# sm00thix/cvmatrix

Hardware: AMD Instinct MI355X
Metric: folds/sec (training_XTX_XTY, center+scale) at N=1e5,K=512 (higher is better)
Workload: dtype f64

## Files before the change

### cvmatrix_amd/csrc/wgram4.hpp

```cpp
#pragma once

constexpr int NT4 = 512;
template <typename T> __device__ __forceinline__ void partial_store(T *p, T v) { *p = v; }
constexpr int NBUF4 = 4;
constexpr size_t LDS4_BYTES = (size_t)NBUF4 * BUF_ELEMS * 8;
template <typename T> constexpr size_t lds4_bytes() { return (size_t)NBUF4 * BUF_ELEMS * sizeof(T); }

__host__ __device__ inline size_t fstat_len(int K, int M);
template <typename T> struct FusedPre;
template <typename T>
__device__ __forceinline__ void fused_g_preload32(FusedPre<T> &p, int a0, int b0, int K, const T *Gt, int lane, int row_lo);
template <typename T, int TP>
__device__ __forceinline__ void fused_finish_direct32(T (*Ts)[TP], const double *rs, int a0, int b0, int K, T *out,
                                                      double swt, bool cX, bool sX, int lane, int row_lo,
                                                      const FusedPre<T> &p);
template <typename T, int TP>
__device__ __forceinline__ void fused_finish_block(T (*Ts)[TP], const double *rs, bool diagb, int a0,
                                                   int b0, int K, const T *Gt, T *out,
                                                   double swt, bool cX, bool sX, int lane);
template <typename T, int TP>
__device__ __forceinline__ void fused_finish_direct(T (*Ts)[TP], const double *rs, bool diagb, int a0,
                                                    int b0, int K, const T *Gt, T *out,
                                                    double swt, bool cX, bool sX, int lane, int row_lo, int row_hi);
template <typename T, int TP>
// ... 96 lines not shown
  else { seg_begin = 0; seg_rows = a.N; }
  int64_t r0, r1;
  split_range(seg_rows, wi.nsp, sp, r0, r1);
  r0 = uni64(r0); r1 = uni64(r1); seg_begin = uni64(seg_begin);
  const int nstages = uni((int)((r1 - r0 + STAGE_ROWS - 1) / STAGE_ROWS));
  const int colA0 = uni(ti * TILE), colB0 = uni(tj * TILE);

  if (ROLER == 3) {
    const int d = wave_all - 4;
    const char *zero_src = reinterpret_cast<const char *>(unip(g_zero_line));
    constexpr unsigned ES = sizeof(T);
    constexpr int EPL = 16 / (int)ES;
    const char *one_src = reinterpret_cast<const char *>(ES == 8 ? (const void *)unip(g_one_line)
                                                                : (const void *)unip(g_one_line_f));
    int oa = EPL * lane, ob = EPL * lane, oy = ES == 8 ? 2 * (lane & 15) : (lane & 31);
    if (colA0 + oa > g.K - EPL) oa = g.K - EPL - colA0;
    if (colB0 + ob > g.K - EPL) ob = g.K - EPL - colB0;
    if (oa < 0) oa = 0;
    if (ob < 0) ob = 0;
    const int ycol0 = yc * YT;
    const int ylast = ES == 8 ? g.M - 2 : g.M - 1;
    if (g.M > 0) { if (ycol0 + oy > ylast) oy = ylast - ycol0; if (oy < 0) oy = 0; } else oy = 0;
    const unsigned va = ES * (unsigned)oa, vb = ES * (unsigned)ob, vy = ES * (unsigned)oy, vw = 4u * (unsigned)lane;
    const unsigned lds0 = (unsigned)(uintptr_t)((__attribute__((address_space(3))) char *)smem_raw);
    auto dma16_all = [&](const char *sbase, unsigned voff, unsigned lds_addr) {
      unsigned keep;
      asm volatile("s_mov_b32 %0, m0\n\ts_mov_b32 m0, %3\n\ts_nop 0\n\t"
                   "global_load_lds_dwordx4 %1, %2\n\ts_mov_b32 m0, %0"
                   : "=&s"(keep) : "v"(voff), "s"(sbase), "s"(lds_addr) : "memory");
    };
    auto dma16_lo16 = [&](const char *sbase, unsigned voff, unsigned lds_addr) {
      unsigned keep; unsigned long long ex;
      asm volatile("s_mov_b32 %0, m0\n\ts_mov_b64 %1, exec\n\ts_mov_b64 exec, 0xffff\n\ts_mov_b32 m0, %4\n\ts_nop 0\n\t"
                   "global_load_lds_dwordx4 %2, %3\n\ts_mov_b64 exec, %1\n\ts_mov_b32 m0, %0"
                   : "=&s"(keep), "=&s"(ex) : "v"(voff), "s"(sbase), "s"(lds_addr) : "memory");
    };
    auto dma16_lo32 = [&](const char *sbase, unsigned voff, unsigned lds_addr) {
      unsigned keep; unsigned long long ex;
      asm volatile("s_mov_b32 %0, m0\n\ts_mov_b64 %1, exec\n\ts_mov_b64 exec, 0xffffffff\n\ts_mov_b32 m0, %4\n\ts_nop 0\n\t"
                   "global_load_lds_dwordx4 %2, %3\n\ts_mov_b64 exec, %1\n\ts_mov_b32 m0, %0"
                   : "=&s"(keep), "=&s"(ex) : "v"(voff), "s"(sbase), "s"(lds_addr) : "memory");
    };
    auto dma4_lo32 = [&](const char *sbase, unsigned voff, unsigned lds_addr) {
      unsigned keep; unsigned long long ex;
      asm volatile("s_mov_b32 %0, m0\n\ts_mov_b64 %1, exec\n\ts_mov_b64 exec, 0xffffffff\n\ts_mov_b32 m0, %4\n\ts_nop 0\n\t"
                   "global_load_lds_dword %2, %3\n\ts_mov_b64 exec, %1\n\ts_mov_b32 m0, %0"
                   : "=&s"(keep), "=&s"(ex) : "v"(voff), "s"(sbase), "s"(lds_addr) : "memory");
    };
    auto dma4_lo1 = [&](const char *sbase, unsigned voff, unsigned lds_addr) {
      unsigned keep; unsigned long long ex;
      asm volatile("s_mov_b32 %0, m0\n\ts_mov_b64 %1, exec\n\ts_mov_b64 exec, 1\n\ts_mov_b32 m0, %4\n\ts_nop 0\n\t"
                   "global_load_lds_dword %2, %3\n\ts_mov_b64 exec, %1\n\ts_mov_b32 m0, %0"
                   : "=&s"(keep), "=&s"(ex) : "v"(voff), "s"(sbase), "s"(lds_addr) : "memory");
    };
    auto dma4_lo2 = [&](const char *sbase, unsigned voff, unsigned lds_addr) {
      unsigned keep; unsigned long long ex;
      asm volatile("s_mov_b32 %0, m0\n\ts_mov_b64 %1, exec\n\ts_mov_b64 exec, 3\n\ts_mov_b32 m0, %4\n\ts_nop 0\n\t"
                   "global_load_lds_dword %2, %3\n\ts_mov_b64 exec, %1\n\ts_mov_b32 m0, %0"
                   : "=&s"(keep), "=&s"(ex) : "v"(voff), "s"(sbase), "s"(lds_addr) : "memory");
    };
    const int r0i = uni((int)r0), r1i = uni((int)r1);
    auto row_numbers = [&](int t, int64_t (&rn)[4], bool (&ok)[4]) {
      int rr[4];
#pragma unroll
      for (int j = 0; j < 4; ++j) {
        rr[j] = r0i + t * STAGE_ROWS + d + 4 * j;
        ok[j] = rr[j] < r1i;
      }
      if (!GATHER) {
#pragma unroll
        for (int j = 0; j < 4; ++j) rn[j] = seg_begin + rr[j];
        return;
      }
      const int64_t *p0 = a.idx + seg_begin + (ok[0] ? rr[0] : 0);
      const int64_t *p1 = a.idx + seg_begin + (ok[1] ? rr[1] : 0);
      const int64_t *p2 = a.idx + seg_begin + (ok[2] ? rr[2] : 0);
      const int64_t *p3 = a.idx + seg_begin + (ok[3] ? rr[3] : 0);
      int64_t v0 = 0, v1 = 0, v2 = 0, v3 = 0;
      if (r1i > 0) {
        asm volatile("s_load_dwordx2 %0, %4, 0x0\n\ts_load_dwordx2 %1, %5, 0x0\n\t"
                     "s_load_dwordx2 %2, %6, 0x0\n\ts_load_dwordx2 %3, %7, 0x0\n\t"
                     "s_waitcnt lgkmcnt(0)"
                     : "=&s"(v0), "=&s"(v1), "=&s"(v2), "=&s"(v3)
                     : "s"(p0), "s"(p1), "s"(p2), "s"(p3) : "memory");
      }
      rn[0] = v0; rn[1] = v1; rn[2] = v2; rn[3] = v3;
    };
    auto issue_stage = [&](int t, const int64_t (&rn)[4], const bool (&ok)[4]) {
      const unsigned bufb = lds0 + (unsigned)((t % NBUF4) * BUF_ELEMS) * ES;
#pragma unroll
      for (int j = 0; j < 4; ++j) {
        const int lrow = d + 4 * j;
        const bool valid = ok[j];
        const char *xrow = reinterpret_cast<const char *>(a.X + rn[j] * (int64_t)g.K);
        const char *pa = valid ? xrow + (int64_t)ES * colA0 : zero_src;
        if (ES == 8) dma16_all(pa, va, bufb + (unsigned)(lrow * PITCH) * ES);
        else dma16_lo32(pa, va, bufb + (unsigned)(lrow * PITCH) * ES);
        if (!diag) {
          const char *pb = valid ? xrow + (int64_t)ES * colB0 : zero_src;
          if (ES == 8) dma16_all(pb, vb, bufb + (unsigned)(PANEL_ELEMS + lrow * PITCH) * ES);
          else dma16_lo32(pb, vb, bufb + (unsigned)(PANEL_ELEMS + lrow * PITCH) * ES);
        } else {
          const char *yrow = (valid && g.M > 0)
              ? reinterpret_cast<const char *>(a.Y + rn[j] * (int64_t)g.M + ycol0) : zero_src;
          if (ES == 8) dma16_lo16(yrow, vy, bufb + (unsigned)(PANEL_ELEMS + lrow * YPITCH) * ES);
          else dma4_lo32(yrow, vy, bufb + (unsigned)(PANEL_ELEMS + lrow * YPITCH) * ES);
        }
        const char *wsrc = valid ? (WEIGHTED ? reinterpret_cast<const char *>(a.w + rn[j]) : one_src) : zero_src;
        if (ES == 8) dma4_lo2(wsrc, vw, bufb + (unsigned)(2 * PANEL_ELEMS + lrow) * ES);
        else dma4_lo1(wsrc, vw, bufb + (unsigned)(2 * PANEL_ELEMS + lrow) * ES);
      }
    };
    auto wait_one_stage_in_flight = [&]() { asm volatile("s_waitcnt vmcnt(12)" ::: "memory"); };
    int64_t rn[4];
    bool ok[4];
#pragma unroll
    for (int t = 0; t < 3; ++t) {
      row_numbers(t, rn, ok);
      issue_stage(t, rn, ok);
    }
    wait_one_stage_in_flight();
    __builtin_amdgcn_s_barrier();
    __builtin_amdgcn_s_barrier();
#ifdef CVM_STAMPS
    unsigned long long t_a = 0, t_b = 0, t_c = 0, t0, t1, t2, t3;
#endif
#pragma unroll 1
    for (int s = 0; s < nstages; ++s) {
#ifdef CVM_STAMPS
      STAMP(t0);
#endif
      row_numbers(s + 3, rn, ok);
      issue_stage(s + 3, rn, ok);
#ifdef CVM_STAMPS
      STAMP(t1);
#endif
      wait_one_stage_in_flight();
#ifdef CVM_STAMPS
      STAMP(t2);
#endif
#ifdef CVM_STAMPS
      if (!(a.dbg & 4))
#endif
      __builtin_amdgcn_s_barrier();
#ifdef CVM_STAMPS
      STAMP(t3);
      t_a += t1 - t0; t_b += t2 - t1; t_c += t3 - t2;
#endif
    }
    asm volatile("s_waitcnt vmcnt(0) lgkmcnt(0)" ::: "memory");
    if constexpr (FUSEDR) {
      if (a.stat_flags && do_g && !diag && d == 0) {
        const int *fl = a.stat_flags + (size_t)seg * g.P;
        fused_wait_flag<T>(fl + ti, fl + tj, smem_raw, lane, seg, uni(xcd_q), uni(slot_q), a.fused_status,
                           a.retry_items, a.retry_mode, a.test_mode);
      }
    }
    if (FUSEDR) lds_barrier();
    if constexpr (FUSEDR) {
      if (do_g && diag && a.stat_flags) {
        __builtin_amdgcn_s_barrier();
        __builtin_amdgcn_s_barrier();
        if (d == 0) {
          const int K = g.K, M = g.M;
          double *fsw = const_cast<double *>(a.fstats) + (size_t)seg * fstat_len(K, M);
          const double *stl = reinterpret_cast<const double *>(smem_raw + diag_tile_bytes<T>()) + 768;
#pragma unroll
          for (int h = 0; h < 2; ++h) {
            const int lcol = 64 * h + lane, col = ti * TILE + lcol;
            if (col < K) { stc(fsw + col, stl[lcol]); stc(fsw + K + col, stl[128 + lcol]); }
          }
          if (lane < 32 && lane < M) { stc(fsw + 2 * K + lane, stl[256 + lane]); stc(fsw + 2 * K + M + lane, stl[288 + lane]); }
          if (lane == 0) stc(fsw + 2 * K + 2 * M, stl[320]);
          asm volatile("s_waitcnt vmcnt(0)" ::: "memory");
          if (lane == 0)
            __hip_atomic_store(a.stat_flags + (size_t)seg * g.P + ti, 1, __ATOMIC_RELAXED, __HIP_MEMORY_SCOPE_AGENT);
        }
      }
      if (do_g && diag && a.out_XTX) {
        constexpr int TP = TILE + 1;
        const int K = g.K, M = g.M;
        const double *fs = a.fstats + (size_t)seg * fstat_len(K, M);
        const double swt = a.stat_flags ? (reinterpret_cast<const double *>(smem_raw + diag_tile_bytes<T>()) + 768)[320]
                                        : ldc(fs + 2 * K + 2 * M);
        const bool cX = a.flags & CVM_CENTER_X, sX = a.flags & CVM_SCALE_X;
        T (*Td)[TP] = reinterpret_cast<T (*)[TP]>(smem_raw);
        double *rs0 = reinterpret_cast<double *>(smem_raw + diag_tile_bytes<T>());
        T *outp = (T *)a.out_XTX + (size_t)(a.seg0 + seg) * (size_t)K * K;
        lds_barrier();
        diag_tile_finish<T, TP>(Td, rs0, wave_all, 0, ti, K, (const T *)a.G, outp, swt, cX, sX, lane);
        lds_barrier();
        diag_tile_finish<T, TP>(Td, rs0, wave_all, 1, ti, K, (const T *)a.G, outp, swt, cX, sX, lane);
      }
      const int mark = (do_g && !diag) ? fused_mark<T>(a.stat_flags, smem_raw) : FUSED_GO;
      if (do_g && !diag && mark != FUSED_SKIP) {
        const int K = g.K, M = g.M;
        const double *fs = a.fstats + (size_t)seg * fstat_len(K, M);
        const double swt = mark == FUSED_POISON ? __builtin_nan("") : ldc(fs + 2 * K + 2 * M);
        const bool cX = a.flags & CVM_CENTER_X, sX = a.flags & CVM_SCALE_X;
        const size_t fo = (size_t)(a.seg0 + seg);
        const int a0 = ti * TILE + 64 * (d >> 1), b0 = tj * TILE + 64 * (d & 1);
        const bool active = a.out_XTX && a0 < K && b0 < K;
        char *slice = smem_raw + (size_t)d * wave_lds_bytes<T>();
        T (*Ts)[65] = reinterpret_cast<T (*)[65]>(slice);
        const double *rs = reinterpret_cast<const double *>(slice + wave_tile_bytes<T>());
        T *outp = (T *)a.out_XTX + fo * (size_t)K * K;
        FusedPre<T> gp;
        if (active) fused_g_preload32<T>(gp, a0, b0, K, (const T *)a.G, lane, 32);
        lds_barrier();
        if (active)
          fused_finish_direct32<T, 65>(Ts, rs, a0, b0, K, outp, swt, cX, sX, lane, 32, gp);
        lds_barrier();
        if (active) fused_finish_mirror<T, 65>(Ts, a0, b0, K, outp, lane, 32, 64);
      }
    }
#ifdef CVM_STAMPS
    if (lane == 0 && blockIdx.x < 1024) {
      unsigned long long *o = g_stamps + ((size_t)blockIdx.x * 8 + wave_all) * 4;
      o[0] = t_a; o[1] = t_b; o[2] = t_c; o[3] = (unsigned long long)nstages;
    }
#endif
    ROLE_EXIT();
  }

  const int stat_role = ROLER;
  acc_t acc[16];
#pragma unroll
  for (int i = 0; i < 16; ++i) acc[i] = (acc_t){0, 0, 0, 0};
  constexpr bool TWO_LEVEL = sizeof(T) == 4;
  acc_t acc2[TWO_LEVEL ? 16 : 1];
  if (TWO_LEVEL) {
#pragma unroll
    for (int i = 0; i < 16; ++i) acc2[i] = (acc_t){0, 0, 0, 0};
  }
  double st_s[4] = {0, 0, 0, 0}, st_q[4] = {0, 0, 0, 0};
  int nz_ = 0, ng_ = 0;

  const int lk = lane >> 4, lc = lane & 15;
  constexpr bool WIDE = !HWR && MFMR && ROLER == 0 && !FUSEDR;
  const int a_col = h_wave ? 0 : (WIDE ? 32 * wave : 64 * wr);
  const int b_col = h_wave ? 0 : (WIDE ? 0 : 64 * wc);
  const int a_off = a_col + lc;
  const int b_off = h_wave ? PANEL_ELEMS + lc : (diag ? 0 : PANEL_ELEMS) + b_col + lc;

  __syncthreads();
  __syncthreads();

#ifdef CVM_STAMPS
  unsigned long long t_a = 0, t_b = 0, t_c = 0, t0, t1, t2, t3;
  unsigned long long c_loop0, c_loop1;
  STAMP(c_loop0);
#endif
  constexpr bool HW = HWR, MFM = MFMR;
  constexpr int ROLE = ROLER;
  constexpr bool TRI = (ROLE == 1) && !HW;
  constexpr int NA = HW ? 8 : (WIDE ? 2 : 4), NB = HW ? 2 : (WIDE ? 8 : 4);
  T af[2][NA], bf[2][NB], yf[2][2], wv[2], raw[4];
  auto read_frags = [&](const T *buf, int ks, int slot) {
    const int r = 4 * ks + lk;
    if (MFM || ROLE == 1) {
#pragma unroll
      for (int m = 0; m < NA; ++m) af[slot][m] = buf[a_off + r * PITCH + 16 * m];
    }
    if (MFM) {
#pragma unroll
      for (int n = 0; n < NB; ++n) bf[slot][n] = buf[b_off + r * (HW ? YPITCH : PITCH) + 16 * n];
    }
    if (ROLE == 2) {
#pragma unroll
      for (int n = 0; n < 2; ++n) yf[slot][n] = buf[PANEL_ELEMS + r * YPITCH + 16 * n + lc];
    }
    wv[slot] = buf[2 * PANEL_ELEMS + r];
  };
  auto prepare = [&](int c) {
    if (ROLE == 1) {
#pragma unroll
      for (int m = 0; m < 4; ++m) {
        raw[m] = af[c][m];
        const T pv = WEIGHTED ? (T)(af[c][m] * wv[c]) : af[c][m];
        st_s[m] += pv; st_q[m] += (T)(pv * raw[m]);
        af[c][m] = pv;
      }
    } else {
      if (ROLE == 2) {
#pragma unroll
        for (int n = 0; n < 2; ++n) {
          const T yv = yf[c][n];
          const T pv = WEIGHTED ? (T)(yv * wv[c]) : yv;
          st_s[n] += pv; st_q[n] += (T)(pv * yv);
        }
        st_s[2] += wv[c];
      }
      if (MFM && WEIGHTED) {
        if (HW) {
#pragma unroll
          for (int n = 0; n < NB; ++n) bf[c][n] *= wv[c];
        } else {
#pragma unroll
          for (int m = 0; m < NA; ++m) af[c][m] *= wv[c];
        }
      }
    }
  };
  if (MFM || ROLE != 0) {
    read_frags(smem, 0, 0);
    prepare(0);
  }
#pragma unroll 1
  for (int sb = 0; sb < nstages; sb += (TWO_LEVEL ? FOLD_STAGES : (1 << 30))) {
  const int se = (TWO_LEVEL && sb + FOLD_STAGES < nstages) ? sb + FOLD_STAGES : nstages;
#pragma unroll 1
  for (int s = sb; s < se; ++s) {
#ifdef CVM_STAMPS
    STAMP(t0);
    STAMP(t1);
    if (a.dbg & 2) { __syncthreads(); continue; }
#endif
    const T *buf = smem + (s % NBUF4) * BUF_ELEMS;
    const T *nbuf = smem + ((s + 1) % NBUF4) * BUF_ELEMS;
    if constexpr (MFM && !HW && ROLE == 0) {
#pragma unroll
      for (int ks = 0; ks < 4; ++ks) {
        const int c = ks & 1;
        const T *rb = ks < 3 ? buf : nbuf;
        const int r = 4 * (ks < 3 ? ks + 1 : 0) + lk;
#pragma unroll
        for (int i = 0; i < 16; ++i) {
          acc[i] = MF<T>::mfma(af[c][i / NB], bf[c][i % NB], acc[i]);
          if (WIDE) {
            if (i == 0) wv[c ^ 1] = rb[2 * PANEL_ELEMS + r];
            else if (i < 3) af[c ^ 1][i - 1] = rb[a_off + r * PITCH + 16 * (i - 1)];
            else if (i < 11) bf[c ^ 1][i - 3] = rb[b_off + r * PITCH + 16 * (i - 3)];
            else if (WEIGHTED && i >= 13 && i < 15) af[c ^ 1][i - 13] *= wv[c ^ 1];
          } else if (i < 4) af[c ^ 1][i] = rb[a_off + r * PITCH + 16 * i];
          else if (i < 8) bf[c ^ 1][i - 4] = rb[b_off + r * PITCH + 16 * (i - 4)];
          else if (i == 8) wv[c ^ 1] = rb[2 * PANEL_ELEMS + r];
          else if (WEIGHTED && i >= 11 && i < 15) af[c ^ 1][i - 11] *= wv[c ^ 1];
          __builtin_amdgcn_sched_barrier(0);
        }
      }
    } else if (MFM || ROLE != 0) {
      T cw = (T)0;
      if (ROLE == 2) cw = buf[2 * PANEL_ELEMS + lc];
#pragma unroll
      for (int ks = 0; ks < 4; ++ks) {
        const int c = ks & 1;
        if (ks < 3) read_frags(buf, ks + 1, c ^ 1); else read_frags(nbuf, 0, c ^ 1);
        __builtin_amdgcn_sched_barrier(0);
        if (MFM) {
#pragma unroll
          for (int m = 0; m < NA / 2; ++m)
#pragma unroll
            for (int n = 0; n < NB; ++n)
              if (!TRI || m <= n) acc[m * NB + n] = MF<T>::mfma(af[c][m], bf[c][n], acc[m * NB + n]);
        }
        __builtin_amdgcn_sched_barrier(0);
        prepare(c ^ 1);
        __builtin_amdgcn_sched_barrier(0);
        if (MFM) {
#pragma unroll
          for (int m = NA / 2; m < NA; ++m)
#pragma unroll
            for (int n = 0; n < NB; ++n)
              if (!TRI || m <= n) acc[m * NB + n] = MF<T>::mfma(af[c][m], bf[c][n], acc[m * NB + n]);
        }
        __builtin_amdgcn_sched_barrier(0);
      }
      if (ROLE == 2) {
        nz_ += __builtin_popcount((unsigned)__builtin_amdgcn_ballot_w64(cw != (T)0) & 0xffffu);
        ng_ += __builtin_popcount((unsigned)__builtin_amdgcn_ballot_w64(cw < (T)0) & 0xffffu);
      }
    }
#ifdef CVM_STAMPS
    STAMP(t2);
    if (!(a.dbg & 4))
#endif
    __syncthreads();
#ifdef CVM_STAMPS
    STAMP(t3);
    t_a += t1 - t0; t_b += t2 - t1; t_c += t3 - t2;
#endif
  }
  if constexpr (TWO_LEVEL) {
    if (se < nstages) {
#pragma unroll
      for (int i = 0; i < 16; ++i) { acc2[i] += acc[i]; acc[i] = (acc_t){0, 0, 0, 0}; }
    }
  }
  }
  if constexpr (TWO_LEVEL) {
#pragma unroll
    for (int i = 0; i < 16; ++i) acc[i] = acc2[i] + acc[i];
  }
#ifdef CVM_STAMPS
  STAMP(c_loop1);
  if (lane == 0 && blockIdx.x < 1024) {
    unsigned long long *o = g_stamps + ((size_t)blockIdx.x * 8 + wave) * 4;
    o[0] = t_a; o[1] = t_b; o[2] = t_c; o[3] = (unsigned long long)nstages;
  }
#endif

  if constexpr (FUSEDR) {
#ifdef CVM_STAMPS
    unsigned long long f0, f1, f2, f3, f4, f5;
    STAMP(f0);
#endif
    __syncthreads();
    const int K = g.K, M = g.M;
    const double *fs = a.fstats + (size_t)seg * fstat_len(K, M);
    const int mark = (do_g && !diag) ? fused_mark<T>(a.stat_flags, smem_raw) : FUSED_GO;
    if (mark == FUSED_SKIP) ROLE_EXIT();
    const double swt = mark == FUSED_POISON ? __builtin_nan("") : ldc(fs + 2 * K + 2 * M);
    const bool cX = a.flags & CVM_CENTER_X, cY = a.flags & CVM_CENTER_Y;
    const bool sX = a.flags & CVM_SCALE_X, sY = a.flags & CVM_SCALE_Y;
    const size_t fo = (size_t)(a.seg0 + seg);
    if (h_wave) {
      if (a.out_XTY && M > 0) {
        T *out = (T *)a.out_XTY + fo * (size_t)K * M;
        const T *Ht = (const T *)a.H;
#pragma unroll
        for (int m = 0; m < 8; ++m)
#pragma unroll
          for (int n = 0; n < 2; ++n)
#pragma unroll
            for (int r = 0; r < 4; ++r) {
              const int row = ti * TILE + 16 * m + MF<T>::drow(lane, r), col = yc * YT + 16 * n + lc;
              if (row < K && col < M) {
                double v = (double)Ht[(size_t)row * M + col] - (double)acc[m * 2 + n][r];
                if (cX || cY) v -= swt * (ldc(fs + row) * ldc(fs + 2 * K + col));
                if (sX && sY) v = v * (ldc(fs + K + row) * ldc(fs + 2 * K + M + col));
                else if (sX) v = v * ldc(fs + K + row);
                else if (sY) v = v * ldc(fs + 2 * K + M + col);
                out[(size_t)row * M + col] = (T)v;
              }
            }
      }
    } else if (do_g && MFM) {
      const int a0 = ti * TILE + 64 * wr, b0 = tj * TILE + 64 * wc;
      const bool active = a.out_XTX && a0 < K && b0 < K;
      char *slice = smem_raw + (size_t)wave * wave_lds_bytes<T>();
      T (*Ts)[65] = reinterpret_cast<T (*)[65]>(slice);
      double *rs = reinterpret_cast<double *>(slice + wave_tile_bytes<T>());
      T *outp = (T *)a.out_XTX + fo * (size_t)K * K;
      FusedPre<T> gp;
      if (active) {
        double r0v = (cX && a0 + lane < K) ? ldc(fs + a0 + lane) : 0.0;
        double r1v = (sX && a0 + lane < K) ? ldc(fs + K + a0 + lane) : 1.0;
        double r2v = (cX && b0 + lane < K) ? ldc(fs + b0 + lane) : 0.0;
        double r3v = (sX && b0 + lane < K) ? ldc(fs + K + b0 + lane) : 1.0;
        if (mark == FUSED_POISON) r0v = r1v = r2v = r3v = __builtin_nan("");
        fused_g_preload32<T>(gp, a0, b0, K, (const T *)a.G, lane, 0);
        rs[lane] = r0v; rs[64 + lane] = r1v; rs[128 + lane] = r2v; rs[192 + lane] = r3v;
#pragma unroll
        for (int m = 0; m < 4; ++m)
#pragma unroll
          for (int n = 0; n < 4; ++n)
#pragma unroll
            for (int r = 0; r < 4; ++r)
              Ts[16 * m + MF<T>::drow(lane, r)][16 * n + lc] = acc[m * 4 + n][r];
      }
#ifdef CVM_STAMPS
      STAMP(f1);
#endif
      lds_barrier();
#ifdef CVM_STAMPS
      STAMP(f2);
#endif
      if (active)
        fused_finish_direct32<T, 65>(Ts, rs, a0, b0, K, outp, swt, cX, sX, lane, 0, gp);
#ifdef CVM_STAMPS
      STAMP(f3);
#endif
      lds_barrier();
#ifdef CVM_STAMPS
      STAMP(f4);
#endif
      if (active) fused_finish_mirror<T, 65>(Ts, a0, b0, K, outp, lane, 0, 32);
#ifdef CVM_STAMPS
      asm volatile("s_waitcnt vmcnt(0)" ::: "memory");
      STAMP(f5);
      if (lane == 0 && wave == 0 && blockIdx.x < 1024) {
        unsigned long long *o = g_stamps4 + (size_t)blockIdx.x * 8;
        o[0] = c_loop0 - c_entry; o[1] = c_loop1 - c_loop0; o[2] = f1 - f0; o[3] = f2 - f1; o[4] = f3 - f2;
        o[5] = f4 - f3; o[6] = f5 - f4; o[7] = f5 - c_entry;
      }
#endif
    }
    ROLE_EXIT();
  }

  auto comb = [&](double v) -> double {
    const double v1 = __shfl(v, lc + 16), v2 = __shfl(v, lc + 32), v3 = __shfl(v, lc + 48);
    return ((v + v1) + v2) + v3;
  };
  if (stat_role == 1) {
    double *st = unit_stats<T>(a.ws, g, u);
#pragma unroll
    for (int m = 0; m < 4; ++m) {
      const double sv = comb(st_s[m]), qv = comb(st_q[m]);
      if (lk == 0) {
        st[ti * TILE + a_col + 16 * m + lc] = sv;
        st[g.Kp + ti * TILE + a_col + 16 * m + lc] = qv;
      }
    }
  } else if (stat_role == 2) {
    double *st = unit_stats<T>(a.ws, g, u);
#pragma unroll
    for (int n = 0; n < 2; ++n) {
      const double sv = comb(st_s[n]), qv = comb(st_q[n]);
      if (lk == 0) {
        st[2 * g.Kp + yc * YT + 16 * n + lc] = sv;
        st[2 * g.Kp + g.Mp + yc * YT + 16 * n + lc] = qv;
      }
    }
    const double swv = comb(st_s[2]);
    if (yc == 0 && lane == 0) {
      st[2 * g.Kp + 2 * g.Mp + 0] = swv;
      st[2 * g.Kp + 2 * g.Mp + 1] = (double)nz_;
      st[2 * g.Kp + 2 * g.Mp + 2] = (double)ng_;
    }
  }
  if (h_wave) {
    if (g.M > 0) {
      T *hp = unit_h<T>(a.ws, g, u) + (size_t)ti * TILE * g.Mp + yc * YT;
#pragma unroll
      for (int m = 0; m < 8; ++m)
#pragma unroll
        for (int n = 0; n < 2; ++n)
#pragma unroll
          for (int r = 0; r < 4; ++r)
            hp[(size_t)(16 * m + MF<T>::drow(lane, r)) * g.Mp + 16 * n + lc] = acc[m * 2 + n][r];
    }
  } else if (do_g) {
    T *tp = unit_tiles<T>(a.ws, g, u) + (size_t)it * TILE * TILE;
    constexpr int SA = (HW || !MFM) ? 4 : NA, SB = (HW || !MFM) ? 4 : NB;
#pragma unroll
    for (int m = 0; m < SA; ++m)
#pragma unroll
      for (int n = 0; n < SB; ++n)
#pragma unroll
        for (int r = 0; r < 4; ++r)
          partial_store(&tp[(a_col + 16 * m + MF<T>::drow(lane, r)) * TILE + b_col + 16 * n + lc], acc[m * SB + n][r]);
  }
#ifdef CVM_STAMPS
  {
    asm volatile("s_waitcnt vmcnt(0)" ::: "memory");
    const unsigned long long c_exit = __builtin_amdgcn_s_memtime();
    if (lane == 0 && blockIdx.x < 1024) {
      unsigned long long *o = g_stamps3 + ((size_t)blockIdx.x * 8 + wave) * 2;
      o[0] = c_loop0 - c_entry; o[1] = c_exit - c_loop1;
    }
    if (lane == 0 && uni(slot_q) < CVM_ITEM_STAMP_STRIDE) {
      unsigned long long *o = g_stamps5 + ((size_t)(uni(xcd_q) * CVM_ITEM_STAMP_STRIDE + uni(slot_q)) * 4 + wave) * 8;
      o[0] = c_entry; o[1] = c_loop0 - c_entry; o[2] = c_loop1 - c_loop0; o[3] = t_b; o[4] = t_c;
      o[5] = (unsigned long long)nstages;
      o[6] = (unsigned long long)(ti | (tj << 8) | (yc << 16)) | ((unsigned long long)blockIdx.x << 32);
      o[7] = c_exit;
    }
  }
#endif
  ROLE_EXIT();
}

struct DiagTab {
  int nf, na, ng, nx;
  int ft[8];
  int at[4];
  int ga[10], gb[10];
  int xa[3];
  int ca[2];
  int rd[8];
  int ys[2];
  int ws;
};
constexpr DiagTab diag_tab_fill(int W, bool strips) {
  DiagTab t{};
  if (!strips) {
    const int R1 = 7 - W;
    t.nf = 8 - W;
    for (int j = 0; j < t.nf; ++j) t.ft[j] = W + j;
    t.na = 2; t.at[0] = 0; t.at[1] = R1 - W;
    t.ng = 9;
    for (int j = 0; j < t.nf; ++j) { t.ga[j] = 0; t.gb[j] = j; }
    for (int j = 0; j < W + 1; ++j) { t.ga[t.nf + j] = 1; t.gb[t.nf + j] = R1 - W + j; }
    t.nx = 2; t.xa[0] = 0; t.xa[1] = 1;
    t.ca[0] = 0; t.ca[1] = 1;
    t.ys[0] = W == 3; t.ys[1] = W == 2; t.ws = W == 1;
    return t;
  }
  t.ys[0] = W == 2; t.ws = W == 3;
  if (W == 0 || W == 3) {
    const int b = W == 0 ? 0 : 4;
    t.nf = 4; t.na = 4;
    for (int j = 0; j < 4; ++j) { t.ft[j] = b + j; t.at[j] = j; }
    t.ng = 0;
    for (int i = 0; i < 4; ++i)
      for (int j = i; j < 4; ++j) { t.ga[t.ng] = i; t.gb[t.ng] = j; ++t.ng; }
    t.nx = 1; t.xa[0] = W == 0 ? 0 : 3;
    t.ca[0] = W == 0 ? 0 : 2; t.ca[1] = W == 0 ? 1 : 3;
    return t;
  }
  const int r = W == 1 ? 0 : 2;
  t.nf = 6;
  t.ft[0] = r; t.ft[1] = r + 1;
  for (int j = 0; j < 4; ++j) t.ft[2 + j] = 4 + j;
  t.ng = 0;
  for (int i = 0; i < 2; ++i)
    for (int j = 0; j < 4; ++j) { t.ga[t.ng] = i; t.gb[t.ng] = 2 + j; ++t.ng; }
  if (W == 1) {
    t.na = 4; t.at[0] = 0; t.at[1] = 1; t.at[2] = 2; t.at[3] = 3;
    t.nx = 3; t.xa[0] = 1; t.xa[1] = 2; t.xa[2] = 3;
    t.ca[0] = 2; t.ca[1] = 3;
  } else {
    t.na = 3; t.at[0] = 0; t.at[1] = 1; t.at[2] = 4;
    t.nx = 3; t.xa[0] = 0; t.xa[1] = 1; t.xa[2] = 2;
    t.ca[0] = 0; t.ca[1] = 1;
  }
  return t;
}
constexpr DiagTab diag_tab(int W, bool strips) {
  DiagTab t = diag_tab_fill(W, strips);
  int n = 0;
  for (int q = 0; q < t.na; ++q) t.rd[n++] = t.at[q];
  for (int j = 0; j < t.nf; ++j) {
    bool is_a = false;
    for (int q = 0; q < t.na; ++q) is_a = is_a || t.at[q] == j;
    if (!is_a) t.rd[n++] = j;
  }
  return t;
}
constexpr bool diag_ystat_wave(int W, int NBY) {
  const DiagTab t = diag_tab(W, NBY == 1);
  return t.ws || t.ys[0] || (NBY > 1 && t.ys[1]);
}

template <typename T, bool WEIGHTED, bool GATHER, int W, int NBY, bool YSTAT, bool FUSEDR = false>
__device__ __noinline__ ROLE_ATTR void wgram4_diag_body(kargs_ptr<T> kargs, int xcd_q, int slot_q) {
  typedef typename MF<T>::acc_t acc_t;
#ifdef CVM_STAMPS
  const unsigned long long c_entry = __builtin_amdgcn_s_memtime();
#endif
  const WgramArgs<T> a = kernel_args<T>(kargs);
  extern __shared__ __attribute__((aligned(16))) char smem_raw[];
  T *smem = reinterpret_cast<T *>(smem_raw);
  const Geom &g = a.g;
  const int lane = threadIdx.x & 63;
  Item wi;
  decode_slot(a, uni(xcd_q), (long)uni(slot_q), wi);
  const long u = wi.u;
  const int it = wi.it, seg = wi.seg, sp = wi.sp, ti = wi.ti;
  int64_t seg_begin, seg_rows;
  if (a.offs) { seg_begin = a.offs[a.seg0 + seg]; seg_rows = a.offs[a.seg0 + seg + 1] - seg_begin; }
  else { seg_begin = 0; seg_rows = a.N; }
  int64_t r0, r1;
  split_range(seg_rows, wi.nsp, sp, r0, r1);
  r0 = uni64(r0); r1 = uni64(r1);
  const int nstages = uni((int)((r1 - r0 + STAGE_ROWS - 1) / STAGE_ROWS));

  constexpr DiagTab P = diag_tab(W, NBY == 1);
  constexpr int NF = P.nf, NA = P.na, NG = P.ng, NX = P.nx;
  acc_t acc[NG], acch[NX * NBY];
#pragma unroll
  for (int i = 0; i < NG; ++i) acc[i] = (acc_t){0, 0, 0, 0};
#pragma unroll
  for (int i = 0; i < NX * NBY; ++i) acch[i] = (acc_t){0, 0, 0, 0};
  constexpr bool TWO_LEVEL = sizeof(T) == 4;
  acc_t acc2[TWO_LEVEL ? NG : 1], acch2[TWO_LEVEL ? NX * NBY : 1];
  if (TWO_LEVEL) {
#pragma unroll
    for (int i = 0; i < NG; ++i) acc2[i] = (acc_t){0, 0, 0, 0};
#pragma unroll
    for (int i = 0; i < NX * NBY; ++i) acch2[i] = (acc_t){0, 0, 0, 0};
  }
  double st_s[2] = {0, 0}, st_q[2] = {0, 0};
  constexpr bool SUMW = YSTAT && P.ws != 0;
  constexpr bool SUMY0 = YSTAT && P.ys[0] != 0, SUMY1 = YSTAT && NBY > 1 && P.ys[1] != 0;
  static_assert(YSTAT == (SUMW || SUMY0 || SUMY1), "a YSTAT instantiation for a wave without Y-side sums");
  double sy[NBY], qy[NBY], sw_ = 0;
  int nz_ = 0, ng_ = 0;
#pragma unroll
  for (int n = 0; n < NBY; ++n) sy[n] = qy[n] = 0;

  const int lk = lane >> 4, lc = lane & 15;
  const bool ink = FUSEDR && a.stat_flags != nullptr;
  double ink_gs[2] = {0, 0}, ink_gq[2] = {0, 0}, ink_tot[2] = {0, 0};
  if (ink) {
#pragma unroll
    for (int q = 0; q < 2; ++q) {
      int col = ti * TILE + 16 * P.ft[P.at[P.ca[q]]] + lc;
      if (col >= g.K) col = g.K - 1;
      ink_gs[q] = a.gstats[col]; ink_gq[q] = a.gstats[g.K + col];
    }
    ink_tot[0] = a.gstats[2 * g.K + 2 * g.M]; ink_tot[1] = a.gstats[2 * g.K + 2 * g.M + 1];
  }
  __syncthreads();
  __syncthreads();
#ifdef CVM_STAMPS
  unsigned long long t_b = 0, t_c = 0, t1, t2, t3, c_loop0, c_loop1;
  STAMP(c_loop0);
#endif

  T bf[2][NF], aw[2][NA], yf[2][NBY], wv[2];
  T cw = (T)0;
  auto read_frags = [&](const T *buf, int ks, int slot) {
    const int r = 4 * ks + lk;
#pragma unroll
    for (int j = 0; j < NF; ++j) bf[slot][j] = buf[r * PITCH + 16 * P.ft[j] + lc];
#pragma unroll
    for (int n = 0; n < NBY; ++n) yf[slot][n] = buf[PANEL_ELEMS + r * YPITCH + 16 * n + lc];
    wv[slot] = buf[2 * PANEL_ELEMS + r];
  };
  auto prepare = [&](int c) {
#pragma unroll
    for (int q = 0; q < NA; ++q) {
      const T x = bf[c][P.at[q]];
      aw[c][q] = WEIGHTED ? (T)(x * wv[c]) : x;
    }
    if (!FUSEDR || ink) {
#pragma unroll
      for (int q = 0; q < 2; ++q) {
        const T x = bf[c][P.at[P.ca[q]]], pv = aw[c][P.ca[q]];
        st_s[q] += pv; st_q[q] += (T)(pv * x);
      }
    }
    if (YSTAT && (!FUSEDR || ink)) {
#pragma unroll
      for (int n = 0; n < NBY; ++n) {
        if (n == 0 ? SUMY0 : SUMY1) {
          const T yv = yf[c][n];
          const T pv = WEIGHTED ? (T)(yv * wv[c]) : yv;
          sy[n] += pv; qy[n] += (T)(pv * yv);
        }
      }
      if (SUMW) sw_ += wv[c];
    }
  };
  auto count_weights = [&]() {
    const unsigned mz = (unsigned)__builtin_amdgcn_ballot_w64(cw != (T)0) & 0xffffu;
    const unsigned mn = (unsigned)__builtin_amdgcn_ballot_w64(cw < (T)0) & 0xffffu;
    nz_ += __builtin_popcount(mz); ng_ += __builtin_popcount(mn);
  };
  auto mfma_i = [&](int i, int c) {
    if (i < NG) acc[i] = MF<T>::mfma(aw[c][P.ga[i]], bf[c][P.gb[i]], acc[i]);
    else {
      const int h = i - NG, x = h / NBY, n = h - x * NBY;
      acch[x * NBY + n] = MF<T>::mfma(aw[c][P.xa[x]], yf[c][n], acch[x * NBY + n]);
    }
  };
  read_frags(smem, 0, 0);
  prepare(0);
#pragma unroll 1
  for (int sb = 0; sb < nstages; sb += (TWO_LEVEL ? FOLD_STAGES : (1 << 30))) {
  const int se = (TWO_LEVEL && sb + FOLD_STAGES < nstages) ? sb + FOLD_STAGES : nstages;
#pragma unroll 1
  for (int s = sb; s < se; ++s) {
    const T *buf = smem + (s % NBUF4) * BUF_ELEMS;
    const T *nbuf = smem + ((s + 1) % NBUF4) * BUF_ELEMS;
#ifdef CVM_STAMPS
    STAMP(t1);
#endif
#pragma unroll
    for (int ks = 0; ks < 4; ++ks) {
      const int c = ks & 1;
      constexpr int NM = NG + NX * NBY;
      constexpr int NR = NF + NBY + 1;
      static_assert(NR <= NM, "more fragment reads than MFMAs in a k-step");
      static_assert(!SUMW || NR < NM, "no MFMA without an LDS read behind it for the weight count");
      const T *rb = ks < 3 ? buf : nbuf;
      const int r = 4 * (ks < 3 ? ks + 1 : 0) + lk;
#pragma unroll
      for (int i = 0; i < NM; ++i) {
        mfma_i(i, c);
        if (i == 0) wv[c ^ 1] = rb[2 * PANEL_ELEMS + r];
        else if (i <= NA) bf[c ^ 1][P.rd[i - 1]] = rb[r * PITCH + 16 * P.ft[P.rd[i - 1]] + lc];
        else if (i <= NA + NBY) yf[c ^ 1][i - NA - 1] = rb[PANEL_ELEMS + r * YPITCH + 16 * (i - NA - 1) + lc];
        else if (i < NR) bf[c ^ 1][P.rd[i - 1 - NBY]] = rb[r * PITCH + 16 * P.ft[P.rd[i - 1 - NBY]] + lc];
        else if (SUMW && i == NR && (!FUSEDR || ink)) {
          if (ks == 0) cw = buf[2 * PANEL_ELEMS + lc];
          else if (ks == 2) count_weights();
        }
        if (i == NM - 1) prepare(c ^ 1);
        __builtin_amdgcn_sched_barrier(0);
      }
    }
#ifdef CVM_STAMPS
    STAMP(t2);
#endif
    __syncthreads();
#ifdef CVM_STAMPS
    STAMP(t3);
    t_b += t2 - t1; t_c += t3 - t2;
#endif
  }
  if constexpr (TWO_LEVEL) {
    if (se < nstages) {
#pragma unroll
      for (int i = 0; i < NG; ++i) { acc2[i] += acc[i]; acc[i] = (acc_t){0, 0, 0, 0}; }
#pragma unroll
      for (int i = 0; i < NX * NBY; ++i) { acch2[i] += acch[i]; acch[i] = (acc_t){0, 0, 0, 0}; }
    }
  }
  }
  if constexpr (TWO_LEVEL) {
#pragma unroll
    for (int i = 0; i < NG; ++i) acc[i] = acc2[i] + acc[i];
#pragma unroll
    for (int i = 0; i < NX * NBY; ++i) acch[i] = acch2[i] + acch[i];
  }
#ifdef CVM_STAMPS
  STAMP(c_loop1);
#endif

  if constexpr (FUSEDR) {
    __syncthreads();
    const int K = g.K, M = g.M;
    double *fsw = const_cast<double *>(a.fstats) + (size_t)seg * fstat_len(K, M);
    const double *fs = fsw;
    const bool cX = a.flags & CVM_CENTER_X, cY = a.flags & CVM_CENTER_Y;
    const bool sX = a.flags & CVM_SCALE_X, sY = a.flags & CVM_SCALE_Y;
    const size_t fo = (size_t)(a.seg0 + seg);
    double *stl = reinterpret_cast<double *>(smem_raw + diag_tile_bytes<T>()) + 768;
    if (ink) {
      auto comb = [&](double v) -> double {
        const double v1 = __shfl(v, lc + 16), v2 = __shfl(v, lc + 32), v3 = __shfl(v, lc + 48);
        return ((v + v1) + v2) + v3;
      };
      double *tot = stl + 322;
      if (SUMW) {
        const double swv = comb(sw_), nzv = (double)nz_;
        if (lane == 0) { tot[0] = swv; tot[1] = nzv; }
      }
      lds_barrier();
      const double swv = tot[0], nzv = tot[1];
      const double swt_ = ink_tot[0] - swv, nzt = ink_tot[1] - nzv;
      const double divisor = (nzt - a.ddof) * swt_ / nzt;
      const bool rXTY = a.flags & CVM_RET_XTY;
      const bool want_muX = cX || sX || (rXTY && cY), want_sdX = sX;
      const bool want_muY = rXTY && (cX || cY || sY), want_sdY = rXTY && sY;
      auto finish_col = [&](double sv, double qv, double gs, double gq, bool want_sd, double &mu, double &isd, double &sd) {
        const double st_ = gs - sv;
        mu = st_ / swt_;
        sd = 1.0;
        if (want_sd) {
          const double qt = gq - qv;
          double var = (-2 * mu * st_ + swt_ * (mu * mu) + qt) / divisor;
// ... 315 lines not shown
```

Baseline: 21420.

## Use paired 16-byte LDS fragment loads and permuted tile stores for f64 wide path

For the f64 wide MFMA path, each lane now reads two adjacent columns with one 128-bit LDS load instead of two scalar loads, using precomputed LDS byte addresses and rebasing them once per stage with an inline add. This permutes which columns each fragment covers, so the partial tile store is rewritten to write paired 8-byte-aligned vectors at the matching permuted positions. The aim is fewer LDS instructions and address computations in the inner MFMA loop. It relies on the column permutation being consistent between load and store, and on the inline asm address update being correct.

```diff
diff --git a/cvmatrix_amd/csrc/wgram4.hpp b/cvmatrix_amd/csrc/wgram4.hpp
--- a/cvmatrix_amd/csrc/wgram4.hpp
+++ b/cvmatrix_amd/csrc/wgram4.hpp
@@ -422,7 +422,26 @@
       }
     }
   };
-  if (MFM || ROLE != 0) {
+  constexpr bool PAIRS = WIDE && sizeof(T) == 8;
+  typedef T pair_t __attribute__((ext_vector_type(2)));
+  typedef const __attribute__((address_space(3))) char *ldsp_t;
+  const unsigned lds0p = (unsigned)(uintptr_t)((__attribute__((address_space(3))) char *)smem_raw);
+  const unsigned oW = lds0p + (unsigned)sizeof(T) * (unsigned)(2 * PANEL_ELEMS + lk);
+  const unsigned oA = lds0p + (unsigned)sizeof(T) * (unsigned)(32 * wave + lk * PITCH + 2 * lc);
+  const unsigned oB = lds0p + (unsigned)sizeof(T) * (unsigned)(PANEL_ELEMS + lk * PITCH + 2 * lc);
+  ldsp_t cW = (ldsp_t)(uintptr_t)oW, cA = (ldsp_t)(uintptr_t)oA, cB = (ldsp_t)(uintptr_t)oB;
+  constexpr int RG = 4 * PITCH * (int)sizeof(T);
+  if constexpr (PAIRS) {
+    wv[0] = *reinterpret_cast<const __attribute__((address_space(3))) T *>(cW);
+    const pair_t ta = *reinterpret_cast<const __attribute__((address_space(3))) pair_t *>(cA);
+    af[0][0] = ta[0]; af[0][1] = ta[1];
+#pragma unroll
+    for (int gq = 0; gq < 4; ++gq) {
+      const pair_t tb = *reinterpret_cast<const __attribute__((address_space(3))) pair_t *>(cB + 256 * gq);
+      bf[0][2 * gq] = tb[0]; bf[0][2 * gq + 1] = tb[1];
+    }
+    prepare(0);
+  } else if (MFM || ROLE != 0) {
     read_frags(smem, 0, 0);
     prepare(0);
   }
@@ -444,10 +463,25 @@
         const int c = ks & 1;
         const T *rb = ks < 3 ? buf : nbuf;
         const int r = 4 * (ks < 3 ? ks + 1 : 0) + lk;
+        const unsigned nb_bytes = (unsigned)(((s + 1) % NBUF4) * BUF_ELEMS) * (unsigned)sizeof(T);
 #pragma unroll
         for (int i = 0; i < 16; ++i) {
           acc[i] = MF<T>::mfma(af[c][i / NB], bf[c][i % NB], acc[i]);
-          if (WIDE) {
+          if constexpr (PAIRS) {
+            const int rs = ks < 3 ? ks + 1 : 0;
+            if (i == 0) wv[c ^ 1] = *reinterpret_cast<const __attribute__((address_space(3))) T *>(cW + 4 * (int)sizeof(T) * rs);
+            else if (i == 1) {
+              const pair_t ta = *reinterpret_cast<const __attribute__((address_space(3))) pair_t *>(cA + RG * rs);
+              af[c ^ 1][0] = ta[0]; af[c ^ 1][1] = ta[1];
+            } else if (i < 6) {
+              const pair_t tb = *reinterpret_cast<const __attribute__((address_space(3))) pair_t *>(cB + RG * rs + 256 * (i - 2));
+              bf[c ^ 1][2 * (i - 2)] = tb[0]; bf[c ^ 1][2 * (i - 2) + 1] = tb[1];
+            } else if (ks == 2 && i < 9) {
+              unsigned x;
+              asm volatile("v_add_u32 %0, %1, %2" : "=v"(x) : "s"(nb_bytes), "v"(i == 6 ? oW : i == 7 ? oA : oB));
+              if (i == 6) cW = (ldsp_t)(uintptr_t)x; else if (i == 7) cA = (ldsp_t)(uintptr_t)x; else cB = (ldsp_t)(uintptr_t)x;
+            } else if (WEIGHTED && i >= 13 && i < 15) af[c ^ 1][i - 13] *= wv[c ^ 1];
+          } else if (WIDE) {
             if (i == 0) wv[c ^ 1] = rb[2 * PANEL_ELEMS + r];
             else if (i < 3) af[c ^ 1][i - 1] = rb[a_off + r * PITCH + 16 * (i - 1)];
             else if (i < 11) bf[c ^ 1][i - 3] = rb[b_off + r * PITCH + 16 * (i - 3)];
@@ -654,6 +688,19 @@
   } else if (do_g) {
     T *tp = unit_tiles<T>(a.ws, g, u) + (size_t)it * TILE * TILE;
     constexpr int SA = (HW || !MFM) ? 4 : NA, SB = (HW || !MFM) ? 4 : NB;
+    if constexpr (PAIRS) {
+      typedef T pair8_t __attribute__((ext_vector_type(2), aligned(8)));
+#pragma unroll
+      for (int m = 0; m < 2; ++m)
+#pragma unroll
+        for (int gq = 0; gq < 4; ++gq)
+#pragma unroll
+          for (int r = 0; r < 4; ++r) {
+            pair8_t v;
+            v[0] = acc[8 * m + 2 * gq][r]; v[1] = acc[8 * m + 2 * gq + 1][r];
+            *reinterpret_cast<pair8_t *>(&tp[(a_col + 2 * MF<T>::drow(lane, r) + m) * TILE + 32 * gq + 2 * lc]) = v;
+          }
+    } else {
 #pragma unroll
     for (int m = 0; m < SA; ++m)
 #pragma unroll
@@ -661,6 +708,7 @@
 #pragma unroll
         for (int r = 0; r < 4; ++r)
           partial_store(&tp[(a_col + 16 * m + MF<T>::drow(lane, r)) * TILE + b_col + 16 * n + lc], acc[m * SB + n][r]);
+    }
   }
 #ifdef CVM_STAMPS
   {
```

After: 21640, median of 6. 1.01x the previous value.
